# peach-xiao/EMRT

Measured on AMD Instinct MI355X. Metric: training tiles/sec at 256x256, higher is better.
Workload: dtype bf16; 1 GPU; EMRT ResNet50, Potsdam 256x256, 6 classes, batch 8 per GPU, fwd+bwd+SGD step (BASELINE configs[1]), bf16; global_batch=8, parallelism=dp1, hipgraph=True

## Files before the change

__graft_entry__.py:

```python
import os
import sys

ROOT = os.path.dirname(os.path.abspath(__file__))
if ROOT not in sys.path:
    sys.path.insert(0, ROOT)


def build():
    from emrt_amd import build_ext
    lib = build_ext.build()
    import emrt_amd
    from emrt_amd import _lib
    L = _lib.lib()
    assert L.query("emrt_abi_version") == 9
    A = _lib.augment_lib()
    assert A.query("emrt_aug_version") == 1
    S = _lib.sampler_lib()
    assert S.query("emrt_smp_version") == 1
    X = _lib.loss_lib()
    assert X.query("emrt_lx_version") == 1
    print("[build] %s: %d entry points" % (os.path.relpath(build_ext.AUG_LIB, ROOT), len(A.protos)))
    print("[build] %s: %d entry points" % (os.path.relpath(build_ext.SMP_LIB, ROOT), len(S.protos)))
    print("[build] %s: %d entry points" % (os.path.relpath(build_ext.LOSS_LIB, ROOT), len(X.protos)))
    print("[build] %s: %d entry points; build mode: %s (%s); inputs sha256 %s" % (
        os.path.relpath(lib, ROOT), len(L.protos), build_ext.LAST_BUILD["mode"],
        ", ".join(build_ext.LAST_BUILD["compiled"]) or "no source changed since the objects were built", build_ext.LAST_BUILD["digest"][:16]))


def smoke():
    import torch
    from emrt_amd.runtime import F32
    from emrt_amd.src.models.emrt import EMRT
    from emrt_amd.src.models.losses import MixSoftmaxCrossEntropyLoss
    from emrt_amd.src.models.solver import Momentum, PolynomialDecay
    from oracle.emrt_torch import EMRT as OracleEMRT

    torch.manual_seed(0)
    ref = OracleEMRT(6, "resnet18").eval()
    model = EMRT(num_classes=6, backbone="resnet18")
    model.load_state_dict(ref.state_dict())
    model.to_hip("cuda:0", F32)
    x = torch.randn(2, 3, 64, 64)
    labels = torch.randint(0, 6, (2, 64, 64))
    model.eval()
    got = model(x.cuda())[0].cpu()
    with torch.no_grad():
        want = ref(x)[0]
    err = (got - want).abs().max().item()
    assert err < 1e-3, "HIP forward differs from the oracle: max |diff| = %g" % err
    assert torch.equal(got.argmax(1), want.argmax(1)), "argmax masks differ from the oracle"
    model.train()
    opt = Momentum(model, PolynomialDecay(0.01, 1000), 0.9, 1e-4, 1.0)
    loss_fn = MixSoftmaxCrossEntropyLoss(ignore_index=255, aux=True, aux_weight=0.4)
    model.clear_gradients()
    loss = loss_fn(model(x.cuda()), labels.cuda())
    loss.backward()
    opt.step()
    torch.cuda.synchronize()
    val = loss.item()
    assert val == val and val > 0, "bad loss %r" % val
    print("[smoke] ok: forward max|diff| vs oracle %.3g, train-step loss %.4f, grad norm %.4f" % (err, val, opt.grad_norm()))


if __name__ == "__main__":
    build()
    if "--smoke" in sys.argv:
        smoke()
```

emrt_amd/_lib.py:

```python
import ctypes
import keyword
import os
import re

_HERE = os.path.dirname(os.path.abspath(__file__))
HEADER = os.path.join(os.path.dirname(_HERE), "include", "emrt_hip.h")
LIB_PATH = os.environ.get("EMRT_HIP_LIB") or os.path.join(_HERE, "csrc", "libemrt_hip.so")

AUG_HEADER = os.path.join(os.path.dirname(_HERE), "include", "emrt_hip_augment.h")
AUG_LIB_PATH = os.environ.get("EMRT_HIP_AUGMENT_LIB") or os.path.join(_HERE, "csrc", "libemrt_hip_augment.so")

SMP_HEADER = os.path.join(os.path.dirname(_HERE), "include", "emrt_hip_sampler.h")
SMP_LIB_PATH = os.environ.get("EMRT_HIP_SAMPLER_LIB") or os.path.join(_HERE, "csrc", "libemrt_hip_sampler.so")

LOSS_HEADER = os.path.join(os.path.dirname(_HERE), "include", "emrt_hip_loss.h")
LOSS_LIB_PATH = os.environ.get("EMRT_HIP_LOSS_LIB") or os.path.join(_HERE, "csrc", "libemrt_hip_loss.so")

_TRACE = bool(int(os.environ.get("EMRT_TRACE", "0")))

_CTYPES = {
    "int": ctypes.c_int, "unsigned": ctypes.c_uint, "float": ctypes.c_float, "double": ctypes.c_double,
    "long long": ctypes.c_longlong, "size_t": ctypes.c_size_t,
}

# ... 248 lines not shown
            setattr(self, "_raw_" + name, fn)
        self._last_error = getattr(self, "_raw_%s_last_error" % prefix)
        version = getattr(self, "_raw_%s_version" % prefix)()
        if version != 1:
            raise EmrtHipError("%s has version %d, this binding expects 1" % (so, version))

    def last_error(self):
        return self._last_error().decode("utf-8", "replace")

    def call(self, name, *args):
        if _TRACE:
            print("[emrt] %s%r" % (name, tuple(a.value if hasattr(a, "value") else a for a in args)), flush=True)
        rc = getattr(self, "_raw_" + name)(*args)
        if rc != 0:
            raise EmrtHipError("%s failed (%d): %s" % (name, rc, self.last_error()))
        if _TRACE:
            import torch
            torch.cuda.synchronize()

    def query(self, name, *args):
        return getattr(self, "_raw_" + name)(*args)


_AUG_LIB = None


def augment_lib():
    global _AUG_LIB
    if _AUG_LIB is None:
        _AUG_LIB = _ExtLib(AUG_LIB_PATH, AUG_HEADER, "emrt_aug", "the device augmentation")
    return _AUG_LIB



_SMP_LIB = None


def sampler_lib():
    global _SMP_LIB
    if _SMP_LIB is None:
        _SMP_LIB = _ExtLib(SMP_LIB_PATH, SMP_HEADER, "emrt_smp", "the class-aware scene sampler")
    return _SMP_LIB



_LOSS_LIB = None


def loss_lib():
    global _LOSS_LIB
    if _LOSS_LIB is None:
        _LOSS_LIB = _ExtLib(LOSS_LIB_PATH, LOSS_HEADER, "emrt_lx", "the Dice + cross-entropy loss")
    return _LOSS_LIB
```

emrt_amd/build_ext.py:

```python
import os
import subprocess
import sys
from concurrent.futures import ThreadPoolExecutor

HERE = os.path.dirname(os.path.abspath(__file__))
CSRC = os.path.join(HERE, "csrc")
LIB = os.path.join(CSRC, "libemrt_hip.so")
SOURCES = ["conv.hip", "norm.hip", "msda.hip", "attn.hip", "spatial.hip", "loss.hip", "optim.hip", "elementwise.hip", "gconv.hip", "augment.hip", "scene.hip"]
HEADER = os.path.join(os.path.dirname(HERE), "include", "emrt_hip.h")
AUG_DIR = os.path.join(CSRC, "augment_ext")
AUG_LIB = os.path.join(CSRC, "libemrt_hip_augment.so")
AUG_SOURCES = ["augment_ext.hip"]
AUG_HEADER = os.path.join(os.path.dirname(HERE), "include", "emrt_hip_augment.h")
SMP_DIR = os.path.join(CSRC, "sampler_ext")
SMP_LIB = os.path.join(CSRC, "libemrt_hip_sampler.so")
SMP_SOURCES = ["sampler_ext.hip"]
SMP_HEADER = os.path.join(os.path.dirname(HERE), "include", "emrt_hip_sampler.h")
GROUPS = [(LIB, CSRC, SOURCES, HEADER), (AUG_LIB, AUG_DIR, AUG_SOURCES, AUG_HEADER), (SMP_LIB, SMP_DIR, SMP_SOURCES, SMP_HEADER)]
LOSS_DIR = os.path.join(CSRC, "loss_ext")
LOSS_LIB = os.path.join(CSRC, "libemrt_hip_loss.so")
LOSS_SOURCES = ["loss_ext.hip"]
LOSS_HEADER = os.path.join(os.path.dirname(HERE), "include", "emrt_hip_loss.h")
EXTRA_GROUPS = [(LOSS_LIB, LOSS_DIR, LOSS_SOURCES, LOSS_HEADER)]
FLAGS = ["--offload-arch=gfx950", "-O3", "-std=c++17", "-fPIC", "-munsafe-fp-atomics", "-Wno-unused-result", "-I../../include"]


def _hipcc():
    for cand in (os.environ.get("HIPCC"), "/opt/rocm/bin/hipcc", "hipcc"):
        if cand and (os.path.isabs(cand) and os.path.exists(cand) or not os.path.isabs(cand)):
            return cand
    return "hipcc"


def _digest(paths, extra=()):
    import hashlib
    h = hashlib.sha256()
    for e in extra:
        h.update(str(e).encode() + b"\0")
    for p in paths:
        h.update(os.path.basename(p).encode() + b"\0")
        with open(p, "rb") as f:
            h.update(f.read())
        h.update(b"\0")
    return h.hexdigest()


def _stamp(target):
    return target + ".inputs"


def _fresh(target, digest):
    try:
        with open(_stamp(target)) as f:
            return os.path.exists(target) and f.read().strip() == digest
    except OSError:
        return False


def all_groups():
    return GROUPS + EXTRA_GROUPS


def _headers():
    return [os.path.join(CSRC, h) for h in sorted(os.listdir(CSRC)) if h.endswith(".hpp")] + [g[3] for g in all_groups()]


def source_digest():
    return _digest([os.path.join(d, s) for _, d, sources, _ in all_groups() for s in sources] + _headers(), [_hipcc()] + FLAGS)


LAST_BUILD = {"mode": None, "digest": None, "compiled": [], "linked": []}


def build(force=False, verbose=True):
    hipcc = _hipcc()
    hdrs = _headers()
    objs, jobs = {g[0]: [] for g in all_groups()}, []
    for lib, d, sources, _ in all_groups():
        for src in sources:
            s = os.path.join(d, src)
            o = os.path.join(d, src.replace(".hip", ".o"))
            objs[lib].append(o)
            dg = _digest([s] + hdrs, [hipcc] + FLAGS)
            if force or not _fresh(o, dg):
                jobs.append(([hipcc] + FLAGS + ["-c", s, "-o", o], o, dg, lib))

    def run(cmd):
        r = subprocess.run(cmd, capture_output=True, text=True, cwd=CSRC)
        if r.returncode != 0:
            raise RuntimeError("hipcc failed: %s\n%s" % (" ".join(cmd), r.stderr[-4000:]))

    def compile_one(job):
        cmd, o, d, _ = job
        if os.path.exists(_stamp(o)):
            os.remove(_stamp(o))
        run(cmd)
        with open(_stamp(o), "w") as f:
            f.write(d + "\n")
        return cmd[-3]

    LAST_BUILD["compiled"] = []
    for lib in {j[3] for j in jobs}:
        if os.path.exists(_stamp(lib)):
            os.remove(_stamp(lib))
    if jobs:
        with ThreadPoolExecutor(max_workers=min(4, len(jobs))) as ex:
            for done in ex.map(compile_one, jobs):
                LAST_BUILD["compiled"].append(os.path.basename(done))
                if verbose:
                    print("[emrt_amd.build] compiled", os.path.basename(done), flush=True)
    total = source_digest()
    linked = LAST_BUILD["linked"] = []
    for lib, _, _, _ in all_groups():
# ... 20 lines not shown
```

emrt_amd/functional.py:

```python
import ctypes
import math

import torch

from . import _lib
from .runtime import ctx, dtype_of, F32


def _L():
    return _lib.lib()


def P(t):
    return None if t is None else ctypes.c_void_p(t.data_ptr())


def _check_map(t):
    assert t.stride(-1) == 1, "inner stride must be 1: %s %s" % (tuple(t.shape), t.stride())
    if t.dim() == 4:
        N, H, W, C = t.shape
        ld = t.stride(2) if W > 1 else (t.stride(1) if H > 1 else (t.stride(0) if N > 1 else C))
        assert H == 1 or W == 1 or t.stride(1) == W * t.stride(2), \
            "expected an NHWC view with dense rows, got shape %s strides %s" % (tuple(t.shape), t.stride())
        return N, H, W, C, ld, (t.stride(0) if N > 1 else H * W * ld)
# ... 6 lines not shown
def _like_shape(t, C):
    return tuple(t.shape[:-1]) + (C,)


def _rows(t):
    C = t.shape[-1]
    assert t.stride(-1) == 1
    ld = t.stride(-2) if t.dim() >= 2 else C
    rows = t.numel() // C
    for d in range(t.dim() - 2):
        assert t.stride(d) == t.stride(d + 1) * t.shape[d + 1], "rows are not uniformly strided: %s %s" % (tuple(t.shape), t.stride())
    return rows, C, ld


def tokens_as_map(t, h, w):
    B, n, C = t.shape
    assert n == h * w
    v = t.as_strided((B, h, w, C), (t.stride(0), w * t.stride(1), t.stride(1), 1), t.storage_offset())
    tape = ctx().tape
    if tape is not None:
        tape.register_alias(v, t, lambda g: g.as_strided((B, h, w, C), (g.stride(0), w * g.stride(1), g.stride(1), 1), g.storage_offset()))
    return v


def map_as_tokens(t):
    B, h, w, C = t.shape
    assert t.stride(1) == w * t.stride(2)
    v = t.as_strided((B, h * w, C), (t.stride(0), t.stride(2), 1), t.storage_offset())
    tape = ctx().tape
    if tape is not None:
        tape.register_alias(v, t, lambda g: g.as_strided((B, h * w, C), (g.stride(0), g.stride(2), 1), g.storage_offset()))
    return v


def view_as(t, shape):
    v = t.view(shape)
    tape = ctx().tape
    if tape is not None:
        tape.register_alias(v, t, lambda g: g.view(shape))
    return v


def param_input(p_data, p_grad):
    c = ctx()
    t = cast_from_f32(p_data)
    tape = c.tape
    if tape is not None:
        def bwd():
            g = tape.pop_grad(t)
            if g is not None:
                add_into(p_grad, cast_to_f32(g))
        tape.record(bwd)
    return t


def narrow(t, dim, start, length):
    v = t.narrow(dim, start, length)
    tape = ctx().tape
    if tape is not None:
        tape.register_alias(v, t, lambda g: g.narrow(dim, start, length))
    return v


def _geom3(*tensors):
    n = tensors[0].numel()
    split = None
    for t in tensors:
        assert t.numel() == n
        if t.dim() >= 2 and not t.is_contiguous():
            N, H, W, C, ld, bs = _check_map(t)
            cur = (N, H * W, C)
            assert split is None or split == cur, "incompatible views %s vs %s" % (split, cur)
            split = cur
    if split is None:
        split = (1, 1, n)
    B, R, Cc = split
    strides = []
    for t in tensors:
        if t.dim() >= 2 and not t.is_contiguous():
            _, _, _, _, ld, bs = _check_map(t)
            strides.append((bs, ld))
        else:
            strides.append((R * Cc, Cc))
    return B, R, Cc, strides


def add_into(dst, src):
    c = ctx()
    assert dst.dtype == src.dtype, (dst.dtype, src.dtype)
    dt = dtype_of(dst)
    B, R, Cc, (sd, ss) = _geom3(dst, src)
    _L().call("emrt_acc3d", P(dst), sd[0], sd[1], P(src), ss[0], ss[1], B, R, Cc, dt, c.stream)


def add(a, b, period=None, bgrad=None):
    c = ctx()
    assert a.is_contiguous() and b.is_contiguous()
    out = c.empty(tuple(a.shape), a.dtype)
    n = a.numel()
    per = n if period is None else period
    dt = dtype_of(a)
    _L().call("emrt_add", P(a), P(b), P(out), n, per, dt, c.stream)
    tape = c.tape
    if tape is not None:
        def bwd():
            g = tape.pop_grad(out)
# ... 1138 lines not shown
    rows = a.numel() // C
    out = c.empty(tuple(a.shape))
    q = None
    if q_pos is not None:
        assert q_pos.is_contiguous() and q_pos.dtype == a.dtype and q_pos.shape[-1] == C and rows % (q_pos.numel() // C) == 0
        q = c.empty(tuple(a.shape))
    keep = c.tape is not None
    p = float(drop_p) if (c.training and b is not None) else 0.0
    z = c.empty(tuple(a.shape)) if (keep and b is not None) else None
    mean = c.empty((rows,), torch.float32) if keep else None
    rstd = c.empty((rows,), torch.float32) if keep else None
    _L().call("emrt_layernorm_fwd", P(a), P(b), P(post), P(z), P(out), P(gamma), P(beta), P(mean), P(rstd), rows, C, eps, p,
              c.seed_ptr if p > 0 else None, drop_salt, P(q_pos) if q is not None else None, (q_pos.numel() // C) if q is not None else 0, P(q),
              c.dtype, c.stream)
    tape = c.tape
    if tape is not None:
        zz = z if z is not None else a

        def bwd():
            dy = tape.pop_grad(out)
            dq = tape.pop_grad(q) if q is not None else None
            if dq is not None:
                assert dq.is_contiguous() and dq.dtype == out.dtype
                if q_bgrad is not None:
                    q_bgrad(dq)
                if dy is None:
                    dy, dq = dq, None
            if dy is None:
                return
            assert dy.is_contiguous()
            dz = c.empty(tuple(a.shape))
            dzb = c.empty(tuple(a.shape)) if (b is not None and p > 0) else None
            ws = c.workspace(_L().query("emrt_layernorm_bwd_workspace_bytes", rows, C))
            dysum = c.empty(tuple(a.shape)) if (dq is not None and post is not None) else None
            extra = tape.peek_grad(identity_from) if identity_from is not None else None
            if extra is not None and (not extra.is_contiguous() or tuple(extra.shape) != tuple(a.shape) or extra.dtype != dz.dtype or (b is not None and dzb is None)):
                extra = None
            _L().call("emrt_layernorm_bwd", P(zz), P(dy), P(dz), P(gamma), P(mean), P(rstd), P(dgamma), P(dbeta), rows, C, P(ws), P(dzb), p,
                      c.seed_ptr if p > 0 else None, drop_salt, P(extra), P(dq), P(dysum), c.dtype, c.stream)
            if extra is not None:
                tape.identity_done[id(identity_from)] = (extra, tape.grad_count(identity_from))
            tape.add_grad(a, dz, owned=(b is None or dzb is not None))
            if b is not None:
                if dzb is not None:
                    tape.add_grad(b, dzb, owned=True)
                else:
                    tape.add_grad(b, dz)
            if post is not None:
                tape.add_grad(post, dy if dysum is None else dysum, owned=dysum is not None)
        tape.record(bwd)
    return out if q is None else (out, q)


def msda(value, offw, ref, shapes, n_heads, n_points, need_dref=False):
    c = ctx()
    B, Lv, CC = value.shape
    M, L, Pn = n_heads, len(shapes), n_points
    assert CC == M * 32 and value.stride(2) == 1
    Lq, ldo = offw.shape[1], offw.shape[2]
    assert offw.is_contiguous() and offw.dtype == torch.float32 and ref.dtype == torch.float32 and ref.is_contiguous()
    ref_L = ref.shape[2]
    assert ref.shape[1] == Lq and ref_L in (1, L) and ref.shape[3] == 2
    ref_bs = 0 if ref.shape[0] == 1 else Lq * ref_L * 2
    arr = (ctypes.c_int * (2 * L))(*[int(v) for hw in shapes for v in hw])
    out = c.empty((B, Lq, CC))
    _L().call("emrt_msda_fwd", P(value), value.stride(1), value.stride(0), P(offw), ldo, P(ref), ref_bs, ref_L, P(out), B, Lq, Lv, M, 32, L, Pn,
              ctypes.cast(arr, ctypes.c_void_p), c.dtype, c.stream)
    tape = c.tape
    if tape is not None:
        def bwd():
            dy = tape.pop_grad(out)
            if dy is None:
                return
            assert dy.is_contiguous()
            odt = None if c.dtype != F32 else torch.float32
            doffw = c.zeros((B, Lq, ldo), odt) if ldo != M * L * Pn * 3 else c.empty((B, Lq, ldo), odt)
            dref = c.zeros((B, Lq, ref_L, 2), torch.float32) if need_dref else None
            dvalue = c.empty((B, Lv, CC))
            ws = c.empty((_L().query("emrt_msda_bwd_workspace_bytes", B, Lq, M, L, Pn, ctypes.cast(arr, ctypes.c_void_p), c.dtype) // 4,), torch.float32)
            _L().call("emrt_msda_bwd", P(value), value.stride(1), value.stride(0), P(offw), ldo, P(ref), ref_bs, ref_L, P(dy), P(dvalue), P(doffw),
                      int(c.dtype != F32), P(dref), B, Lq, Lv, M, 32, L, Pn, ctypes.cast(arr, ctypes.c_void_p), P(ws), ws.numel() * 4, c.dtype, c.stream)
            tape.add_grad(value, dvalue, owned=True)
            tape.add_grad(offw, doffw, owned=True)
            if need_dref:
                if ref.shape[0] == 1 and B > 1:
                    red = c.zeros((1, Lq, ref_L, 2), torch.float32)
                    colsum_acc(dref.view(B, Lq * ref_L * 2), red.view(-1))
                    dref = red
                tape.add_grad(ref, dref)
        tape.record(bwd)
    return out


def mha(qk, v, n_heads, pdrop, salt):
    c = ctx()
    B, L, E2 = qk.shape
    E = E2 // 2
    assert qk.is_contiguous() and v.is_contiguous() and E == n_heads * 32
    out = c.empty((B, L, E))
    probs = c.empty((B, n_heads, L, L), torch.float32)
    p = float(pdrop) if c.training else 0.0
    scale = 1.0 / math.sqrt(32.0)
    q_ptr = qk.data_ptr()
    k_ptr = qk.data_ptr() + E * qk.element_size()
    path = ctypes.c_int(-1)
    _L().call("emrt_mha_fwd", ctypes.c_void_p(q_ptr), E2, ctypes.c_void_p(k_ptr), E2, P(v), E, P(out), E, P(probs), B, n_heads, L, 32, scale, p,
              c.seed_ptr, salt, ctypes.pointer(path), c.dtype, c.stream)
    tape = c.tape
    if tape is not None:
        def bwd():
            dy = tape.pop_grad(out)
            if dy is None:
                return
            assert dy.is_contiguous()
            dqk = c.empty((B, L, E2))
            dv = c.empty((B, L, E))
            _L().call("emrt_mha_bwd", ctypes.c_void_p(q_ptr), E2, ctypes.c_void_p(k_ptr), E2, P(v), E, P(probs), P(dy), E,
                      ctypes.c_void_p(dqk.data_ptr()), E2, ctypes.c_void_p(dqk.data_ptr() + E * dqk.element_size()), E2, P(dv), E,
                      B, n_heads, L, 32, scale, p, c.seed_ptr, salt, path.value, c.dtype, c.stream)
            tape.add_grad(qk, dqk, owned=True)
            tape.add_grad(v, dv, owned=True)
        tape.record(bwd)
    return out


def nchw_to_nhwc(img, c_out=None):
    c = ctx()
    N, C, H, W = img.shape
    assert img.dtype == torch.float32 and img.is_contiguous()
    co = C if c_out is None else int(c_out)
    out = c.empty((N, H, W, co))
    _L().call("emrt_nchw_to_nhwc", P(img), P(out), N, C, H, W, co, c.dtype, c.stream)
    return out


def resize_bilinear(x, OH, OW, align_corners, add_t=None, out=None, out_nchw_f32=False):
    c = ctx()
# ... 372 lines not shown
```

emrt_amd/runtime.py:

```python
import ctypes

import torch

from . import _lib

F32, BF16, F16 = 0, 1, 2
_TORCH_DTYPE = {F32: torch.float32, BF16: torch.bfloat16, F16: torch.float16}
_DTYPE_OF_TORCH = {v: k for k, v in _TORCH_DTYPE.items()}


def dtype_of(t):
    return _DTYPE_OF_TORCH[t.dtype]


class Tape:
    def __init__(self):
        self.ops = []
        self.stash = None
        self.grads = {}
        self.keep = []
        self.alias = {}
        self.watched = {}
        self.results = {}
        self.splits = []
# ... 142 lines not shown
            _CTX.wgrad_join()
        finally:
            _CTX._in_backward = False
        if stop_at > 0:
            return
        self.results = {k: self.grad(t) for k, t in self.watched.items()}
        self.ops = []
        self.grads = {}
        self.keep = []
        self.alias = {}
        self.identity_done = {}


class Context:
    def __init__(self):
        self.dtype = F32
        self.tape = None
        self.training = False
        self.device = None
        self._ws = None
        self._seed = None
        self.step_counter = None
        self.world_size = 1
        self.sync_bn = True
        self.salt_counter = 0
        self.keepalive = None
        self._arena = None
        self._arena_off = 0
        self._arena_live = False
        self.overlap = False
        self._side = None
        self._in_backward = False
        self._main = None
        self.fold_eval_bn = True
        self.fold_live = False
        self.capture = None
        self.sync_always = False
        import os
        self.wgrad_batch = int(os.environ.get("EMRT_WGRAD_BATCH", "24"))
        self.bn_defer = bool(int(os.environ.get("EMRT_BN_DEFER", "1")))
        self.bn_conv = bool(int(os.environ.get("EMRT_BN_CONV", "1")))
        self.bn_small_group = bool(int(os.environ.get("EMRT_BN_SMALL_GROUP", "1")))
        self.conv_pair = bool(int(os.environ.get("EMRT_CONV_PAIR", "1")))
        self.side_branch = bool(int(os.environ.get("EMRT_SIDE_BRANCH", "1")))
        self.side = None
        self.dgrad_pair = bool(int(os.environ.get("EMRT_DGRAD_PAIR", "1")))
        self.side_host_tiles = int(os.environ.get("EMRT_SIDE_HOST_TILES", "128"))
        self.segment_order = False
        self.head_pair = bool(int(os.environ.get("EMRT_HEAD_PAIR", "1")))
        self.enc_front = bool(int(os.environ.get("EMRT_ENC_FRONT", "1")))
        self.group_attn_proj = bool(int(os.environ.get("EMRT_GROUP_ATTN_PROJ", "1")))
        self.fuse_ffn_dropout = bool(int(os.environ.get("EMRT_FFN_DROPOUT_FUSED", "1")))
        self.ln_query = bool(int(os.environ.get("EMRT_LN_QUERY", "1")))
        self.pyramid_group = bool(int(os.environ.get("EMRT_PYRAMID_GROUP", "1")))
        self.wgrad_side = bool(int(os.environ.get("EMRT_WGRAD_SIDE", "0")))
        self._wside = None
        self._wside_keep = []
        self.prologue_side = bool(int(os.environ.get("EMRT_PROLOGUE_SIDE", "0")))
        self._pside = None
        self._prologue_pending = False
        self.pack_bwd_done = False

    def collective(self, fn):
        self.prologue_join()
        if self.capture is not None:
            self.capture.interlude(fn)
        else:
            fn()

    def prologue_stream(self):
        if self._pside is None:
            self._pside = torch.cuda.Stream(device=self.device)
        self._pside.wait_stream(torch.cuda.current_stream())
        self._prologue_pending = True
        return self._pside

    def prologue_join(self):
        if self._prologue_pending:
            torch.cuda.current_stream().wait_stream(self._pside)
            self._prologue_pending = False

    def fork(self, *keep):
        if not self.overlap:
            return None
        if self._side is None:
            self._side = torch.cuda.Stream(device=self.device)
            self._side_keep = []
        self._side.wait_stream(torch.cuda.current_stream())
        if self.overlap == "deferred":
            self._side_keep.extend(keep)
        return ctypes.c_void_p(self._side.cuda_stream)

    def join(self):
        if self.overlap == "pair":
            torch.cuda.current_stream().wait_stream(self._side)

    def join_all(self):
        if self._side is not None:
            torch.cuda.current_stream().wait_stream(self._side)
            self._side_keep = []
        self.wgrad_join()

    def wgrad_fork(self, keep):
        if self._wside is None:
            self._wside = torch.cuda.Stream(device=self.device)
        self._wside.wait_stream(torch.cuda.current_stream())
# ... 133 lines not shown
```

emrt_amd/src/models/emrt.py:

```python
import ctypes
import math

import torch
import torch.nn as tnn

from ... import functional as Fn
from ... import nn as hnn
from ...runtime import ctx, Tape, F32

NOGRAD_PARAMS = ("backbone.fc.weight", "backbone.fc.bias", "model.tgt_embed.weight", "backbone.out.weight", "backbone.out.bias")
IMAGE_CHANNELS = 8

LATE_GRAD_PREFIXES = ("backbone.conv1.", "backbone.bn1.", "backbone.layer1.", "backbone.layer2.", "backbone.layer3.")
GRAD_SEGMENT_PREFIXES = (("backbone.layer3.",), ("backbone.conv1.", "backbone.bn1.", "backbone.layer1.", "backbone.layer2."))


def _salt():
    return ctx().next_salt()


class BasicBlock(hnn.HipLayer):
    expansion = 1

    def __init__(self, inplanes, planes, stride=1, downsample=None):
# ... 220 lines not shown
    def __init__(self, in_channels, channels, num_classes, dropout_ratio=0.1, up_ratio=16):
        super().__init__()
        self.up_ratio, self.p = up_ratio, dropout_ratio
        self.convs = hnn.Sequential(hnn.Sequential(hnn.Conv2D(in_channels, channels, 3, 1, 1, bias=False),
                                                   hnn.BatchNorm2D(channels, sync=True), None))
        self.conv_seg = hnn.Conv2D(channels, num_classes, 1)
        self.salt = _salt()

    def forward(self, x, features=None):
        N, H, W, _ = x.shape
        o = features if features is not None else Fn.conv_bn(self.convs[0][0], self.convs[0][1], x, relu=True)
        o = Fn.dropout(o, self.p, self.salt, mode=1, hw=H * W, sole_consumer_is_linear=True)
        o = self.conv_seg(o)
        return Fn.resize_bilinear(o, H * self.up_ratio, W * self.up_ratio, False, out_nchw_f32=True)


class MSDeformableAttention(hnn.HipLayer):
    def __init__(self, embed_dim=256, num_heads=8, num_levels=3, num_points=6):
        super().__init__()
        self.embed_dim, self.num_heads, self.num_levels, self.num_points = embed_dim, num_heads, num_levels, num_points
        tp = num_heads * num_levels * num_points
        self.total_points = tp
        self.sampling_offsets = hnn.Linear(embed_dim, tp * 2)
        self.attention_weights = hnn.Linear(embed_dim, tp)
        self.value_proj = hnn.Linear(embed_dim, embed_dim)
        self.output_proj = hnn.Linear(embed_dim, embed_dim)
        self.sampling_offsets.standalone = False
        self.attention_weights.standalone = False
        self.offw_gemm = None
        self._reset_parameters()

    @torch.no_grad()
    def _reset_parameters(self):
        tnn.init.zeros_(self.sampling_offsets.weight)
        thetas = torch.arange(self.num_heads, dtype=torch.float32) * (2.0 * math.pi / self.num_heads)
        grid = torch.stack([thetas.cos(), thetas.sin()], -1)
        grid = grid / grid.abs().max(-1, keepdim=True)[0]
        grid = grid.reshape(self.num_heads, 1, 1, 2).repeat(1, self.num_levels, self.num_points, 1)
        grid = grid * torch.arange(1, self.num_points + 1, dtype=torch.float32).reshape(1, 1, -1, 1)
        self.sampling_offsets.bias.copy_(grid.flatten())
        tnn.init.zeros_(self.attention_weights.weight)
        tnn.init.zeros_(self.attention_weights.bias)
        tnn.init.xavier_uniform_(self.value_proj.weight)
        tnn.init.zeros_(self.value_proj.bias)
        tnn.init.xavier_uniform_(self.output_proj.weight)
        tnn.init.zeros_(self.output_proj.bias)

    def bind(self, store, prefix):
        ow, ob = store.offsets[prefix + "sampling_offsets.weight"], store.offsets[prefix + "sampling_offsets.bias"]
        assert store.offsets[prefix + "attention_weights.weight"] == ow + self.total_points * 2 * self.embed_dim
        assert store.offsets[prefix + "attention_weights.bias"] == ob + self.total_points * 2
        self.offw_gemm = store.make_gemm(ow, self.total_points * 3, self.embed_dim, 1, 1, ob)

    def forward(self, query, reference_points, value, spatial_shapes, need_dref=False, projected=None):
        c = ctx()
        if projected is not None:
            value, offw = projected
        elif c.group_attn_proj and value.dim() == 3 and query.dim() == 3 and value.is_contiguous() and query.is_contiguous() and value is not query:
            value, offw = Fn.linear_group([(value, self.value_proj.gw, False), (query, self.offw_gemm, True)])
        else:
            value = self.value_proj(value)
            offw = Fn.linear(query, self.offw_gemm, out_f32=True)
        out = Fn.msda(value, offw, reference_points, spatial_shapes, self.num_heads, self.num_points, need_dref=need_dref)
        return self.output_proj(out)


class MultiHeadAttention(hnn.HipLayer):
    def __init__(self, embed_dim, num_heads, dropout=0.0):
        super().__init__()
        self.embed_dim, self.num_heads, self.dropout = embed_dim, num_heads, dropout
        self.in_proj_weight = tnn.Parameter(torch.empty(3 * embed_dim, embed_dim))
        self.in_proj_bias = tnn.Parameter(torch.zeros(3 * embed_dim))
        self.out_proj = hnn.Linear(embed_dim, embed_dim)
        self.salt = _salt()
        with torch.no_grad():
            bound = math.sqrt(6.0 / (embed_dim + 3 * embed_dim))
            self.in_proj_weight.uniform_(-bound, bound)
            tnn.init.xavier_uniform_(self.out_proj.weight)
            tnn.init.zeros_(self.out_proj.bias)

    def bind(self, store, prefix):
        E = self.embed_dim
        w, b = store.offsets[prefix + "in_proj_weight"], store.offsets[prefix + "in_proj_bias"]
        self.qk_gemm = store.make_gemm(w, 2 * E, E, 1, 1, b)
        self.v_gemm = store.make_gemm(w + 2 * E * E, E, E, 1, 1, b + 2 * E)

    def forward(self, qk_in, v_in):
        if ctx().group_attn_proj and qk_in.is_contiguous() and v_in.is_contiguous() and qk_in.dim() == 3:
            qk, v = Fn.linear_group([(qk_in, self.qk_gemm, False), (v_in, self.v_gemm, False)])
        else:
            qk = Fn.linear(qk_in, self.qk_gemm)
            v = Fn.linear(v_in, self.v_gemm)
        out = Fn.mha(qk, v, self.num_heads, self.dropout, self.salt)
        return self.out_proj(out)


def _linear_init_(m):
    bound = 1 / math.sqrt(m.weight.shape[1])
    tnn.init.uniform_(m.weight, -bound, bound)
    tnn.init.uniform_(m.bias, -bound, bound)


@torch.no_grad()
def _paddle_conv_default_(conv):
    fan = conv.weight.shape[1] * conv.weight.shape[2] * conv.weight.shape[3]
    conv.weight.normal_(0.0, math.sqrt(2.0 / fan))
    if conv.bias is not None:
        conv.bias.zero_()


class TransformerEncoderLayer(hnn.HipLayer):
    def __init__(self, d_model=256, n_head=8, dim_feedforward=1024, dropout=0.1, n_levels=3, n_points=6):
        super().__init__()
        self.p = dropout
        self.self_attn = MSDeformableAttention(d_model, n_head, n_levels, n_points)
        self.norm1 = hnn.LayerNorm(d_model)
# ... 24 lines not shown
                q = Fn.add(src, pos, period=Lv * C, bgrad=pos_bgrad)
            lin = [(src, self.self_attn.value_proj.gw, False), (q, self.self_attn.offw_gemm, True)]
            if c.enc_front and c.group_attn_proj and q.is_contiguous() and q is not src and Fn.level_conv_gn_takes_linears(src, gws, lin):
                src_flatten, projected = Fn.level_conv_gn(src, gws, gns, spatial_shapes, level_spans, linears=lin)
            else:
                src_flatten = Fn.level_conv_gn(src, gws, gns, spatial_shapes, level_spans)
            identity = src_flatten
        else:
            identity = None
            src_flatten = ctx().empty((B, Lv, C))
            for (h, w), (s0, n), seq in zip(spatial_shapes, level_spans, seqs):
                x_l = Fn.tokens_as_map(Fn.narrow(src, 1, s0, n), h, w)
                y = seq[0](x_l)
                seq[1](y, gelu=True, residual=x_l, out=Fn.tokens_as_map(Fn.narrow(src_flatten, 1, s0, n), h, w))
        if q is None:
            q = Fn.add(src, pos, period=Lv * C, bgrad=pos_bgrad)
        src2 = self.self_attn(q, reference_points, src, spatial_shapes, projected=projected)
        src = self.norm1(src, src2, drop_p=self.p, drop_salt=self.salts[0], identity_from=identity)
        h1 = self.linear1(src, relu=True, drop=(self.p, self.salts[1]))
        ff = self.linear2(h1)
        return self.norm2(src, ff, post=src_flatten, drop_p=self.p, drop_salt=self.salts[2], q_pos=pos if next_q else None, q_bgrad=pos_bgrad)


class TransformerEncoder(hnn.HipLayer):
    def __init__(self, make_layer, num_layers):
        super().__init__()
        first = make_layer()
        layers = [first]
        for _ in range(1, num_layers):
            lyr = make_layer()
            lyr.load_state_dict(first.state_dict())
            layers.append(lyr)
        self.layers = tnn.ModuleList(layers)


class TransformerDecoderLayer(hnn.HipLayer):
    def __init__(self, d_model=256, n_head=8, dim_feedforward=1024, dropout=0.1, n_levels=3, n_points=6):
        super().__init__()
        self.p = dropout
        self.self_attn = MultiHeadAttention(d_model, n_head, dropout=dropout)
        self.norm1 = hnn.LayerNorm(d_model)
        self.cross_attn = MSDeformableAttention(d_model, n_head, n_levels, n_points)
        self.norm2 = hnn.LayerNorm(d_model)
        self.linear1 = hnn.Linear(d_model, dim_feedforward)
        self.linear2 = hnn.Linear(dim_feedforward, d_model)
        self.norm3 = hnn.LayerNorm(d_model)
        self.salts = [_salt(), _salt(), _salt(), _salt()]
        with torch.no_grad():
            _linear_init_(self.linear1)
            _linear_init_(self.linear2)
            tnn.init.xavier_uniform_(self.linear1.weight)
            tnn.init.xavier_uniform_(self.linear2.weight)

    def forward(self, tgt, reference_points, memory, spatial_shapes, query_pos, qpos_bgrad, q=None, next_q=False):
        Lq, C = tgt.shape[1], tgt.shape[2]
        fuse = ctx().ln_query
        if q is None:
            q = Fn.add(tgt, query_pos, period=Lq * C, bgrad=qpos_bgrad)
        if fuse:
            tgt, q2 = self.norm1(tgt, self.self_attn(q, tgt), drop_p=self.p, drop_salt=self.salts[0], q_pos=query_pos, q_bgrad=qpos_bgrad)
        else:
            tgt = self.norm1(tgt, self.self_attn(q, tgt), drop_p=self.p, drop_salt=self.salts[0])
            q2 = Fn.add(tgt, query_pos, period=Lq * C, bgrad=qpos_bgrad)
        tgt2 = self.cross_attn(q2, reference_points, memory, spatial_shapes, need_dref=True)
        tgt = self.norm2(tgt, tgt2, drop_p=self.p, drop_salt=self.salts[1])
        h1 = self.linear1(tgt, relu=True, drop=(self.p, self.salts[2]))
        return self.norm3(tgt, self.linear2(h1), drop_p=self.p, drop_salt=self.salts[3], q_pos=query_pos if next_q else None, q_bgrad=qpos_bgrad)


class TransformerDecoder(hnn.HipLayer):
    def __init__(self, make_layer, num_layers):
        super().__init__()
        first = make_layer()
        layers = [first]
        for _ in range(1, num_layers):
            lyr = make_layer()
            lyr.load_state_dict(first.state_dict())
            layers.append(lyr)
        self.layers = tnn.ModuleList(layers)


def sine_position_embedding(h, w, num_pos_feats=128, temperature=10000, offset=-0.5, eps=1e-6, scale=2 * math.pi):
    y_embed = torch.arange(1, h + 1, dtype=torch.float32).reshape(h, 1).expand(h, w)
    x_embed = torch.arange(1, w + 1, dtype=torch.float32).reshape(1, w).expand(h, w)
    y_embed = (y_embed + offset) / (y_embed[-1:, :] + eps) * scale
    x_embed = (x_embed + offset) / (x_embed[:, -1:] + eps) * scale
    dim_t = 2 * (torch.arange(num_pos_feats) // 2).to(torch.float32)
    dim_t = temperature ** (dim_t / num_pos_feats)
    pos_x = x_embed.unsqueeze(-1) / dim_t
    pos_y = y_embed.unsqueeze(-1) / dim_t
    pos_x = torch.stack((pos_x[:, :, 0::2].sin(), pos_x[:, :, 1::2].cos()), dim=3).flatten(2)
    pos_y = torch.stack((pos_y[:, :, 0::2].sin(), pos_y[:, :, 1::2].cos()), dim=3).flatten(2)
    return torch.cat((pos_y, pos_x), dim=2).reshape(h * w, 2 * num_pos_feats)


def encoder_reference_points(spatial_shapes):
    pts = []
    for (H, W) in spatial_shapes:
        ref_y, ref_x = torch.meshgrid(torch.linspace(0.5, H - 0.5, H), torch.linspace(0.5, W - 0.5, W), indexing="ij")
        pts.append(torch.stack((ref_x.flatten() / W, ref_y.flatten() / H), dim=-1))
    return torch.cat(pts, 0).reshape(1, -1, 1, 2).contiguous()


class EncoderDecoder(hnn.HipLayer):
    def __init__(self, num_queries=110, backbone_num_channels=(512, 1024, 2048), num_feature_levels=3,
                 num_encoder_points=6, num_decoder_points=6, hidden_dim=256, nhead=8, num_encoder_layers=4,
                 num_decoder_layers=2, dim_feedforward=1024, dropout=0.1):
        super().__init__()
        self.hidden_dim, self.nhead, self.num_queries = hidden_dim, nhead, num_queries
        self.encoder = TransformerEncoder(lambda: TransformerEncoderLayer(hidden_dim, nhead, dim_feedforward, dropout,
                                                                          num_feature_levels, num_encoder_points), num_encoder_layers)
        self.decoder = TransformerDecoder(lambda: TransformerDecoderLayer(hidden_dim, nhead, dim_feedforward, dropout,
                                                                          num_feature_levels, num_decoder_points), num_decoder_layers)
        self.level_embed = hnn.Embedding(num_feature_levels, hidden_dim)
        self.tgt_embed = hnn.Embedding(num_queries, hidden_dim)
        self.query_pos_embed = hnn.Embedding(num_queries, hidden_dim)
        self.reference_points = hnn.Linear(hidden_dim, 2)
# ... 27 lines not shown
        spans, s0 = [], 0
        for h, w in spatial_shapes:
            spans.append((s0, h * w))
            s0 += h * w
        Lv = s0
        if all(f.is_contiguous() and n <= 4096 for f, (_, n) in zip(src_feats, spans)) and len(src_feats) <= 4:
            src, _ = Fn.level_proj_gn(list(src_feats), [p_[0].gw for p_ in self.input_proj],
                                      [(p_[1].weight.data, p_[1].bias.data, p_[1].weight.grad, p_[1].bias.grad) for p_ in self.input_proj])
        else:
            src = c.empty((B, Lv, C))
            for f, (h, w), (a, n), proj in zip(src_feats, spatial_shapes, spans, self.input_proj):
                y = proj[0](f)
                proj[1](y, out=Fn.tokens_as_map(Fn.narrow(src, 1, a, n), h, w))
        sine, ref_enc = self._constants(spatial_shapes)
        pos = c.empty((Lv, C))
        lvl = self.level_embed.weight
        if len(spans) <= 4 and lvl.data.is_contiguous():
            starts = (ctypes.c_int * len(spans))(*[a for a, _ in spans])
            Fn._L().call("emrt_add_f32row_levels", Fn.P(sine), Fn.P(lvl.data), Fn.P(pos), starts, len(spans), Lv, C, c.dtype, c.stream)
        else:
            for l, (a, n) in enumerate(spans):
                Fn._L().call("emrt_add_f32row", Fn.P(sine[a:a + n]), Fn.P(lvl.data[l]), Fn.P(pos[a:a + n]), n * C, C, c.dtype, c.stream)

        pos_acc = []

        def pos_bgrad(g):
            pos_acc.append(g)

        if c.tape is not None:
            def pos_reduce():
                if not pos_acc:
                    return
                if (len(pos_acc) <= 8 and len(spans) <= 4 and all(g.is_contiguous() and tuple(g.shape) == (B, Lv, C) and g.dtype == pos_acc[0].dtype for g in pos_acc)
                        and lvl.grad.is_contiguous() and C % 4 == 0 and 256 % (C // 4) == 0):
                    ptrs = (ctypes.c_void_p * len(pos_acc))(*[g.data_ptr() for g in pos_acc])
                    st_ = (ctypes.c_int * len(spans))(*[a for a, _ in spans])
                    cn_ = (ctypes.c_int * len(spans))(*[n for _, n in spans])
                    Fn._L().call("emrt_colsum_levels_multi", ptrs, len(pos_acc), st_, cn_, len(spans), B, Lv, C, Fn.P(lvl.grad), Fn.dtype_of(pos_acc[0]), c.stream)
                else:
                    for g in pos_acc:
                        for l, (a, n) in enumerate(spans):
                            Fn.colsum_acc(g.narrow(1, a, n), lvl.grad[l])
                pos_acc.clear()
            c.tape.record(pos_reduce)

        memory, q = src, None
        n_enc = len(self.encoder.layers)
        for i, layer in enumerate(self.encoder.layers):
            nq = c.ln_query and i + 1 < n_enc
            res = layer(memory, ref_enc, spatial_shapes, spans, pos, pos_bgrad, q=q, next_q=nq)
            memory, q = res if nq else (res, None)

        qpe = self.query_pos_embed.weight
        query_pos = Fn.param_input(qpe.data, qpe.grad)

        def qpos_bgrad(g):
            Fn.colsum_acc(g.reshape(g.shape[0], -1), qpe.grad.view(-1))

        ref_logit = self.reference_points(query_pos, out_f32=True)
        ref_dec = Fn.view_as(Fn.sigmoid_f32(ref_logit), (1, self.num_queries, 1, 2))
        tgt, q = src_psp, None
        n_dec = len(self.decoder.layers)
        for i, layer in enumerate(self.decoder.layers):
            nq = c.ln_query and i + 1 < n_dec
            res = layer(tgt, ref_dec, memory, spatial_shapes, query_pos, qpos_bgrad, q=q, next_q=nq)
            tgt, q = res if nq else (res, None)
        return tgt, memory, spatial_shapes, spans


class Conv2dBlock(hnn.HipLayer):
    def __init__(self, cin, cout):
        super().__init__()
        self.conv1 = hnn.Sequential(hnn.Conv2D(cin, cout, 3, 1, 1, bias=False), hnn.BatchNorm2D(cout), None)
        self.conv2 = hnn.Sequential(hnn.Conv2D(cout, cout, 3, 1, 1, bias=False), hnn.BatchNorm2D(cout), None)

    def forward(self, x):
        o = Fn.conv_bn(self.conv1[0], self.conv1[1], x, relu=True, defer="conv")
        o = Fn.conv_bn(self.conv2[0], self.conv2[1], o, relu=True)
        return Fn.add_maps(o, x)


class EFP(hnn.HipLayer):
    def __init__(self, cin=256, cout=256):
        super().__init__()
        self.conv0, self.conv1, self.conv2 = Conv2dBlock(cin, cout), Conv2dBlock(cin, cout), Conv2dBlock(cin, cout)

    def forward(self, x0, x1, x2, out):
        blocks, xs = (self.conv0, self.conv1, self.conv2), (x0, x1, x2)
        c1, b1 = [b.conv1[0] for b in blocks], [b.conv1[1] for b in blocks]
        c2, b2 = [b.conv2[0] for b in blocks], [b.conv2[1] for b in blocks]
        if Fn._small_group_ok(c1, b1, xs):
            mid = Fn.conv_bn_small_group(c1, b1, xs, relu=True)
            if Fn._small_group_ok(c2, b2, mid, post_adds=xs):
                o0, o1, o2 = Fn.conv_bn_small_group(c2, b2, mid, relu=True, post_adds=xs)
            else:
                o0, o1, o2 = [Fn.add_maps(Fn.conv_bn(cv, b, m_, relu=True), x) for cv, b, m_, x in zip(c2, b2, mid, xs)]
            x21 = Fn.resize_bilinear(o2, x1.shape[1], x1.shape[2], True, add_t=o1)
            return Fn.resize_bilinear(x21, x0.shape[1], x0.shape[2], True, add_t=o0, out=out)
        o2 = self.conv2(x2)
        o1 = self.conv1(x1)
        x21 = Fn.resize_bilinear(o2, x1.shape[1], x1.shape[2], True, add_t=o1)
        o0 = self.conv0(x0)
        return Fn.resize_bilinear(x21, x0.shape[1], x0.shape[2], True, add_t=o0, out=out)


class PyramidPoolingModule(hnn.HipLayer):
    def __init__(self, pool_scales, in_channels, channels):
        super().__init__()
        self.pool_scales = list(pool_scales)
        self.pool_branches = tnn.ModuleList([
            hnn.Sequential(None, hnn.Conv2D(in_channels, channels, 1, bias=False), hnn.BatchNorm2D(channels, sync=True), None)
            for _ in pool_scales])

    def forward(self, x, extra=None):
        tokens = Fn.adaptive_avgpool_tokens(x, self.pool_scales)
        slices, s0 = [], 0
        for k in self.pool_scales:
            slices.append(Fn.narrow(tokens, 1, s0, k * k))
# ... 249 lines not shown
```

Baseline: 1011 tiles/s.

## Fuse decoder query-pos cast, reference-point linear and sigmoid into one kernel

Adds a new HIP extension that, in one forward kernel, casts the query-position embedding, computes the 2-wide reference-point projection and applies the sigmoid. The backward pass collects the query-pos gradient slabs and MSDA reference-point gradients from all decoder layers and reduces them in one kernel, instead of a colsum per layer plus separate linear and sigmoid backward passes. It is meant to remove several small launches and the per-layer dref reductions. The cost is more code, buffered gradient lists that flush when full, and a fallback path for unsupported shapes.

Result: no change. 1018 tiles/s (median of 6 runs) (+0.7%).

```diff
diff --git a/__graft_entry__.py b/__graft_entry__.py
--- a/__graft_entry__.py
+++ b/__graft_entry__.py
@@ -19,9 +19,12 @@
     assert S.query("emrt_smp_version") == 1
     X = _lib.loss_lib()
     assert X.query("emrt_lx_version") == 1
+    Y = _lib.query_lib()
+    assert Y.query("emrt_qp_version") == 1
     print("[build] %s: %d entry points" % (os.path.relpath(build_ext.AUG_LIB, ROOT), len(A.protos)))
     print("[build] %s: %d entry points" % (os.path.relpath(build_ext.SMP_LIB, ROOT), len(S.protos)))
     print("[build] %s: %d entry points" % (os.path.relpath(build_ext.LOSS_LIB, ROOT), len(X.protos)))
+    print("[build] %s: %d entry points" % (os.path.relpath(build_ext.QUERY_LIB, ROOT), len(Y.protos)))
     print("[build] %s: %d entry points; build mode: %s (%s); inputs sha256 %s" % (
         os.path.relpath(lib, ROOT), len(L.protos), build_ext.LAST_BUILD["mode"],
         ", ".join(build_ext.LAST_BUILD["compiled"]) or "no source changed since the objects were built", build_ext.LAST_BUILD["digest"][:16]))
diff --git a/emrt_amd/_lib.py b/emrt_amd/_lib.py
--- a/emrt_amd/_lib.py
+++ b/emrt_amd/_lib.py
@@ -324,3 +324,17 @@
     if _LOSS_LIB is None:
         _LOSS_LIB = _ExtLib(LOSS_LIB_PATH, LOSS_HEADER, "emrt_lx", "the Dice + cross-entropy loss")
     return _LOSS_LIB
+
+
+
+QUERY_HEADER = os.path.join(os.path.dirname(_HERE), "include", "emrt_hip_query.h")
+QUERY_LIB_PATH = os.environ.get("EMRT_HIP_QUERY_LIB") or os.path.join(_HERE, "csrc", "libemrt_hip_query.so")
+
+_QUERY_LIB = None
+
+
+def query_lib():
+    global _QUERY_LIB
+    if _QUERY_LIB is None:
+        _QUERY_LIB = _ExtLib(QUERY_LIB_PATH, QUERY_HEADER, "emrt_qp", "the decoder's query parameters")
+    return _QUERY_LIB
diff --git a/emrt_amd/build_ext.py b/emrt_amd/build_ext.py
--- a/emrt_amd/build_ext.py
+++ b/emrt_amd/build_ext.py
@@ -22,6 +22,11 @@
 LOSS_SOURCES = ["loss_ext.hip"]
 LOSS_HEADER = os.path.join(os.path.dirname(HERE), "include", "emrt_hip_loss.h")
 EXTRA_GROUPS = [(LOSS_LIB, LOSS_DIR, LOSS_SOURCES, LOSS_HEADER)]
+QUERY_DIR = os.path.join(CSRC, "query_ext")
+QUERY_LIB = os.path.join(CSRC, "libemrt_hip_query.so")
+QUERY_SOURCES = ["query_ext.hip"]
+QUERY_HEADER = os.path.join(os.path.dirname(HERE), "include", "emrt_hip_query.h")
+MORE_GROUPS = [(QUERY_LIB, QUERY_DIR, QUERY_SOURCES, QUERY_HEADER)]
 FLAGS = ["--offload-arch=gfx950", "-O3", "-std=c++17", "-fPIC", "-munsafe-fp-atomics", "-Wno-unused-result", "-I../../include"]
 
 
@@ -58,7 +63,7 @@
 
 
 def all_groups():
-    return GROUPS + EXTRA_GROUPS
+    return GROUPS + EXTRA_GROUPS + MORE_GROUPS
 
 
 def _headers():
diff --git a/emrt_amd/csrc/query_ext/query_ext.hip b/emrt_amd/csrc/query_ext/query_ext.hip
--- /dev/null
+++ b/emrt_amd/csrc/query_ext/query_ext.hip
@@ -0,0 +1,173 @@
+#include "../common.hpp"
+#include "../../../include/emrt_hip_query.h"
+
+namespace emrt {
+namespace {
+
+thread_local char g_qp_err[512] = "";
+
+int qp_fail(const char* fn, const char* msg) {
+  snprintf(g_qp_err, sizeof(g_qp_err), "%s: %s", fn, msg);
+  return -1;
+}
+int qp_check_launch(const char* fn) {
+  hipError_t e = hipGetLastError();
+  if (e != hipSuccess) {
+    snprintf(g_qp_err, sizeof(g_qp_err), "%s: launch failed: %s", fn, hipGetErrorString(e));
+    return -2;
+  }
+  return 0;
+}
+#define QP_REQUIRE(cond, msg)                     \
+  do {                                            \
+    if (!(cond)) return qp_fail(__func__, msg);   \
+  } while (0)
+
+}
+
+template <class T>
+__device__ __forceinline__ float rounded(float x) { return to_f32(from_f32<T>(x)); }
+
+template <class T>
+__global__ __launch_bounds__(256) void qp_prep_fwd_kernel(const float* __restrict__ embed, const float* __restrict__ weight, const float* __restrict__ bias,
+                                                          T* __restrict__ query_pos, float* __restrict__ ref, int Q, int C) {
+  const int lane = threadIdx.x & 63, q = blockIdx.x * 4 + (threadIdx.x >> 6);
+  if (q >= Q) return;
+  float a0 = 0.f, a1 = 0.f;
+  for (int c = lane; c < C; c += 64) {
+    const T xt = from_f32<T>(embed[(size_t)q * C + c]);
+    query_pos[(size_t)q * C + c] = xt;
+    const float x = to_f32(xt);
+    a0 = fmaf(x, rounded<T>(weight[c]), a0);
+    a1 = fmaf(x, rounded<T>(weight[C + c]), a1);
+  }
+  a0 = wave_sum(a0);
+  a1 = wave_sum(a1);
+  if (lane < 2) {
+    const float z = (lane ? a1 : a0) + (bias ? bias[lane] : 0.f);
+    ref[q * 2 + lane] = 1.f / (1.f + expf(-z));
+  }
+}
+
+template <class T>
+struct QpBwd {
+  const T* slab[EMRT_QP_MAX_SLABS];
+  const float* dref[EMRT_QP_MAX_DREF];
+  int nslabs, ndref;
+  const float* ref;
+  const T* query_pos;
+  const float* weight;
+  float *d_embed, *d_weight, *d_bias;
+  int B, Q, C, row_blocks;
+};
+
+template <class T>
+__device__ __forceinline__ float qp_dlogit(const QpBwd<T>& a, int q, int j) {
+  float s = 0.f;
+  for (int k = 0; k < a.ndref; ++k)
+    for (int b = 0; b < a.B; ++b) s += a.dref[k][((size_t)b * a.Q + q) * 2 + j];
+  const float r = a.ref[q * 2 + j];
+  return s * r * (1.f - r);
+}
+
+template <class T>
+__global__ __launch_bounds__(256) void qp_prep_bwd_kernel(QpBwd<T> a) {
+  __shared__ float dl[EMRT_QP_MAX_QUERIES * 2];
+  __shared__ float part[4][2][64];
+  const int lane = threadIdx.x & 63, wv = threadIdx.x >> 6;
+  const int Q = a.Q, C = a.C;
+  if ((int)blockIdx.x < a.row_blocks) {
+    const int q = blockIdx.x * 4 + wv;
+    if (q >= Q) return;
+    const float d0 = qp_dlogit(a, q, 0), d1 = qp_dlogit(a, q, 1);
+    for (int c = lane * 4; c < C; c += 256) {
+      float acc[4] = {0.f, 0.f, 0.f, 0.f};
+      for (int s = 0; s < a.nslabs; ++s) {
+        const T* g = a.slab[s] + (size_t)q * C + c;
+#pragma unroll 4
+        for (int b = 0; b < a.B; ++b) {
+          float v[4];
+          Vec4<T>::load(g + (size_t)b * Q * C, v);
+#pragma unroll
+          for (int e = 0; e < 4; ++e) acc[e] += v[e];
+        }
+      }
+#pragma unroll
+      for (int e = 0; e < 4; ++e) {
+        float t = fmaf(d0, rounded<T>(a.weight[c + e]), acc[e]);
+        t = fmaf(d1, rounded<T>(a.weight[C + c + e]), t);
+        a.d_embed[(size_t)q * C + c + e] += t;
+      }
+    }
+    return;
+  }
+  for (int i = threadIdx.x; i < 2 * Q; i += 256) dl[i] = qp_dlogit(a, i >> 1, i & 1);
+  __syncthreads();
+  const int c = ((int)blockIdx.x - a.row_blocks) * 64 + lane;
+  float w0 = 0.f, w1 = 0.f;
+  if (c < C) {
+    for (int q = wv; q < Q; q += 4) {
+      const float x = to_f32(a.query_pos[(size_t)q * C + c]);
+      w0 = fmaf(dl[q * 2], x, w0);
+      w1 = fmaf(dl[q * 2 + 1], x, w1);
+    }
+  }
+  part[wv][0][lane] = w0;
+  part[wv][1][lane] = w1;
+  __syncthreads();
+  if (wv < 2 && c < C)
+    a.d_weight[(size_t)wv * C + c] += ((part[0][wv][lane] + part[1][wv][lane]) + part[2][wv][lane]) + part[3][wv][lane];
+  if ((int)blockIdx.x == a.row_blocks && wv == 2 && a.d_bias) {
+    float b0 = 0.f, b1 = 0.f;
+    for (int q = lane; q < Q; q += 64) { b0 += dl[q * 2]; b1 += dl[q * 2 + 1]; }
+    b0 = wave_sum(b0);
+    b1 = wave_sum(b1);
+    if (lane < 2) a.d_bias[lane] += lane ? b1 : b0;
+  }
+}
+
+}
+
+using namespace emrt;
+
+extern "C" const char* emrt_qp_last_error(void) { return g_qp_err; }
+extern "C" int emrt_qp_version(void) { return 1; }
+
+extern "C" int emrt_qp_prep_fwd(const float* embed, const float* weight, const float* bias, void* query_pos, float* ref, int Q, int C, int dtype, void* stream) {
+  QP_REQUIRE(dtype == EMRT_F32 || dtype == EMRT_BF16 || dtype == EMRT_F16, "dtype must be 0 (float32), 1 (bfloat16) or 2 (float16)");
+  QP_REQUIRE(embed && weight && query_pos && ref, "null pointer");
+  QP_REQUIRE(Q >= 1 && Q <= EMRT_QP_MAX_QUERIES && C >= 1 && C <= 65536, "1 <= Q <= 2048 and 1 <= C <= 65536");
+  const dim3 grid((unsigned)((Q + 3) / 4));
+  hipStream_t st = (hipStream_t)stream;
+  if (dtype == EMRT_F32) hipLaunchKernelGGL(qp_prep_fwd_kernel<float>, grid, dim3(256), 0, st, embed, weight, bias, (float*)query_pos, ref, Q, C);
+  else if (dtype == EMRT_BF16) hipLaunchKernelGGL(qp_prep_fwd_kernel<bf16_t>, grid, dim3(256), 0, st, embed, weight, bias, (bf16_t*)query_pos, ref, Q, C);
+  else hipLaunchKernelGGL(qp_prep_fwd_kernel<f16_t>, grid, dim3(256), 0, st, embed, weight, bias, (f16_t*)query_pos, ref, Q, C);
+  return qp_check_launch("emrt_qp_prep_fwd");
+}
+
+template <class T>
+static int qp_backward(const void* const* slabs, int nslabs, const float* const* drefs, int ndref, const float* ref, const void* query_pos, const float* weight,
+                       float* d_embed, float* d_weight, float* d_bias, int B, int Q, int C, void* stream) {
+  QpBwd<T> a;
+  for (int s = 0; s < EMRT_QP_MAX_SLABS; ++s) a.slab[s] = s < nslabs ? (const T*)slabs[s] : nullptr;
+  for (int s = 0; s < EMRT_QP_MAX_DREF; ++s) a.dref[s] = s < ndref ? drefs[s] : nullptr;
+  a.nslabs = nslabs; a.ndref = ndref; a.ref = ref; a.query_pos = (const T*)query_pos; a.weight = weight;
+  a.d_embed = d_embed; a.d_weight = d_weight; a.d_bias = d_bias;
+  a.B = B; a.Q = Q; a.C = C; a.row_blocks = (Q + 3) / 4;
+  hipLaunchKernelGGL(qp_prep_bwd_kernel<T>, dim3((unsigned)(a.row_blocks + (C + 63) / 64)), dim3(256), 0, (hipStream_t)stream, a);
+  return qp_check_launch("emrt_qp_prep_bwd");
+}
+
+extern "C" int emrt_qp_prep_bwd(const void* slabs, int nslabs, const void* drefs, int ndref, const float* ref, const void* query_pos, const float* weight,
+                                float* d_embed, float* d_weight, float* d_bias, int B, int Q, int C, int dtype, void* stream) {
+  QP_REQUIRE(dtype == EMRT_F32 || dtype == EMRT_BF16, "dtype must be 0 (float32) or 1 (bfloat16): float16 is inference-only");
+  QP_REQUIRE(nslabs >= 0 && nslabs <= EMRT_QP_MAX_SLABS && ndref >= 0 && ndref <= EMRT_QP_MAX_DREF, "0..8 gradient slabs and 0..4 reference-point gradients");
+  QP_REQUIRE((slabs || nslabs == 0) && (drefs || ndref == 0) && ref && query_pos && weight && d_embed && d_weight, "null pointer");
+  QP_REQUIRE(B >= 1 && Q >= 1 && Q <= EMRT_QP_MAX_QUERIES && C >= 4 && C <= 65536 && C % 4 == 0, "B >= 1, 1 <= Q <= 2048, 4 <= C <= 65536 and C % 4 == 0");
+  const void* const* sl = (const void* const*)slabs;
+  const float* const* dr = (const float* const*)drefs;
+  for (int s = 0; s < nslabs; ++s) QP_REQUIRE(sl[s] && ((uintptr_t)sl[s]) % 16 == 0, "every gradient slab must be a 16-byte aligned device pointer");
+  for (int s = 0; s < ndref; ++s) QP_REQUIRE(dr[s], "null reference-point gradient");
+  if (dtype == EMRT_F32) return qp_backward<float>(sl, nslabs, dr, ndref, ref, query_pos, weight, d_embed, d_weight, d_bias, B, Q, C, stream);
+  return qp_backward<bf16_t>(sl, nslabs, dr, ndref, ref, query_pos, weight, d_embed, d_weight, d_bias, B, Q, C, stream);
+}
diff --git a/emrt_amd/functional.py b/emrt_amd/functional.py
--- a/emrt_amd/functional.py
+++ b/emrt_amd/functional.py
@@ -82,6 +82,43 @@
                 add_into(p_grad, cast_to_f32(g))
         tape.record(bwd)
     return t
+
+
+def query_prep(embed, weight, bias):
+    c = ctx()
+    Q, C = embed.data.shape
+    assert tuple(weight.data.shape) == (2, C) and embed.data.is_contiguous() and weight.data.is_contiguous()
+    X = _lib.query_lib()
+    query_pos = c.empty((Q, C))
+    ref = c.empty((Q, 2), torch.float32)
+    X.call("emrt_qp_prep_fwd", P(embed.data), P(weight.data), P(bias.data if bias is not None else None), P(query_pos), P(ref), Q, C, c.dtype, c.stream)
+    slabs, drefs = [], []
+    tape = c.tape
+    if tape is not None:
+        def flush():
+            B = (slabs[0] if slabs else drefs[0]).shape[0]
+            assert all(g.is_contiguous() and tuple(g.shape) == (B, Q, C) and g.dtype == query_pos.dtype for g in slabs)
+            assert all(d.is_contiguous() and tuple(d.shape) == (B, Q, 1, 2) and d.dtype == torch.float32 for d in drefs)
+            sp = (ctypes.c_void_p * max(len(slabs), 1))(*[g.data_ptr() for g in slabs])
+            dp = (ctypes.c_void_p * max(len(drefs), 1))(*[d.data_ptr() for d in drefs])
+            X.call("emrt_qp_prep_bwd", sp, len(slabs), dp, len(drefs), P(ref), P(query_pos), P(weight.data), P(embed.grad), P(weight.grad),
+                   P(bias.grad if bias is not None else None), B, Q, C, c.dtype, c.stream)
+            slabs.clear()
+            drefs.clear()
+
+        def add(lst, cap):
+            def sink(g):
+                if len(lst) == cap:
+                    flush()
+                lst.append(g)
+            return sink
+
+        def bwd():
+            if slabs or drefs:
+                flush()
+        tape.record(bwd)
+        return query_pos, ref, add(slabs, 8), add(drefs, 4)
+    return query_pos, ref, None, None
 
 
 def narrow(t, dim, start, length):
@@ -1326,7 +1363,7 @@
     return out if q is None else (out, q)
 
 
-def msda(value, offw, ref, shapes, n_heads, n_points, need_dref=False):
+def msda(value, offw, ref, shapes, n_heads, n_points, need_dref=False, dref_sink=None):
     c = ctx()
     B, Lv, CC = value.shape
     M, L, Pn = n_heads, len(shapes), n_points
@@ -1356,7 +1393,9 @@
                       int(c.dtype != F32), P(dref), B, Lq, Lv, M, 32, L, Pn, ctypes.cast(arr, ctypes.c_void_p), P(ws), ws.numel() * 4, c.dtype, c.stream)
             tape.add_grad(value, dvalue, owned=True)
             tape.add_grad(offw, doffw, owned=True)
-            if need_dref:
+            if need_dref and dref_sink is not None:
+                dref_sink(dref)
+            elif need_dref:
                 if ref.shape[0] == 1 and B > 1:
                     red = c.zeros((1, Lq, ref_L, 2), torch.float32)
                     colsum_acc(dref.view(B, Lq * ref_L * 2), red.view(-1))
diff --git a/emrt_amd/runtime.py b/emrt_amd/runtime.py
--- a/emrt_amd/runtime.py
+++ b/emrt_amd/runtime.py
@@ -218,6 +218,7 @@
         self.group_attn_proj = bool(int(os.environ.get("EMRT_GROUP_ATTN_PROJ", "1")))
         self.fuse_ffn_dropout = bool(int(os.environ.get("EMRT_FFN_DROPOUT_FUSED", "1")))
         self.ln_query = bool(int(os.environ.get("EMRT_LN_QUERY", "1")))
+        self.query_prep = bool(int(os.environ.get("EMRT_QUERY_PREP", "1")))
         self.pyramid_group = bool(int(os.environ.get("EMRT_PYRAMID_GROUP", "1")))
         self.wgrad_side = bool(int(os.environ.get("EMRT_WGRAD_SIDE", "0")))
         self._wside = None
diff --git a/emrt_amd/src/models/emrt.py b/emrt_amd/src/models/emrt.py
--- a/emrt_amd/src/models/emrt.py
+++ b/emrt_amd/src/models/emrt.py
@@ -296,7 +296,7 @@
         assert store.offsets[prefix + "attention_weights.bias"] == ob + self.total_points * 2
         self.offw_gemm = store.make_gemm(ow, self.total_points * 3, self.embed_dim, 1, 1, ob)
 
-    def forward(self, query, reference_points, value, spatial_shapes, need_dref=False, projected=None):
+    def forward(self, query, reference_points, value, spatial_shapes, need_dref=False, projected=None, dref_sink=None):
         c = ctx()
         if projected is not None:
             value, offw = projected
@@ -305,7 +305,7 @@
         else:
             value = self.value_proj(value)
             offw = Fn.linear(query, self.offw_gemm, out_f32=True)
-        out = Fn.msda(value, offw, reference_points, spatial_shapes, self.num_heads, self.num_points, need_dref=need_dref)
+        out = Fn.msda(value, offw, reference_points, spatial_shapes, self.num_heads, self.num_points, need_dref=need_dref, dref_sink=dref_sink)
         return self.output_proj(out)
 
 
@@ -436,7 +436,7 @@
             tnn.init.xavier_uniform_(self.linear1.weight)
             tnn.init.xavier_uniform_(self.linear2.weight)
 
-    def forward(self, tgt, reference_points, memory, spatial_shapes, query_pos, qpos_bgrad, q=None, next_q=False):
+    def forward(self, tgt, reference_points, memory, spatial_shapes, query_pos, qpos_bgrad, q=None, next_q=False, dref_sink=None):
         Lq, C = tgt.shape[1], tgt.shape[2]
         fuse = ctx().ln_query
         if q is None:
@@ -446,7 +446,7 @@
         else:
             tgt = self.norm1(tgt, self.self_attn(q, tgt), drop_p=self.p, drop_salt=self.salts[0])
             q2 = Fn.add(tgt, query_pos, period=Lq * C, bgrad=qpos_bgrad)
-        tgt2 = self.cross_attn(q2, reference_points, memory, spatial_shapes, need_dref=True)
+        tgt2 = self.cross_attn(q2, reference_points, memory, spatial_shapes, need_dref=True, dref_sink=dref_sink)
         tgt = self.norm2(tgt, tgt2, drop_p=self.p, drop_salt=self.salts[1])
         h1 = self.linear1(tgt, relu=True, drop=(self.p, self.salts[2]))
         return self.norm3(tgt, self.linear2(h1), drop_p=self.p, drop_salt=self.salts[3], q_pos=query_pos if next_q else None, q_bgrad=qpos_bgrad)
@@ -580,18 +580,25 @@
             memory, q = res if nq else (res, None)
 
         qpe = self.query_pos_embed.weight
-        query_pos = Fn.param_input(qpe.data, qpe.grad)
-
-        def qpos_bgrad(g):
-            Fn.colsum_acc(g.reshape(g.shape[0], -1), qpe.grad.view(-1))
-
-        ref_logit = self.reference_points(query_pos, out_f32=True)
-        ref_dec = Fn.view_as(Fn.sigmoid_f32(ref_logit), (1, self.num_queries, 1, 2))
+        rp = self.reference_points
+        dref_sink = None
+        if (c.query_prep and C % 4 == 0 and self.num_queries <= 2048 and qpe.data.is_cuda and qpe.data.is_contiguous() and rp.weight.data.is_contiguous()
+                and rp.bias is not None):
+            query_pos, ref, qpos_bgrad, dref_sink = Fn.query_prep(qpe, rp.weight, rp.bias)
+            ref_dec = ref.view(1, self.num_queries, 1, 2)
+        else:
+            query_pos = Fn.param_input(qpe.data, qpe.grad)
+
+            def qpos_bgrad(g):
+                Fn.colsum_acc(g.reshape(g.shape[0], -1), qpe.grad.view(-1))
+
+            ref_logit = rp(query_pos, out_f32=True)
+            ref_dec = Fn.view_as(Fn.sigmoid_f32(ref_logit), (1, self.num_queries, 1, 2))
         tgt, q = src_psp, None
         n_dec = len(self.decoder.layers)
         for i, layer in enumerate(self.decoder.layers):
             nq = c.ln_query and i + 1 < n_dec
-            res = layer(tgt, ref_dec, memory, spatial_shapes, query_pos, qpos_bgrad, q=q, next_q=nq)
+            res = layer(tgt, ref_dec, memory, spatial_shapes, query_pos, qpos_bgrad, q=q, next_q=nq, dref_sink=dref_sink)
             tgt, q = res if nq else (res, None)
         return tgt, memory, spatial_shapes, spans
 
diff --git a/include/emrt_hip_query.h b/include/emrt_hip_query.h
--- /dev/null
+++ b/include/emrt_hip_query.h
@@ -0,0 +1,23 @@
+#ifndef EMRT_HIP_QUERY_H
+#define EMRT_HIP_QUERY_H
+#include <stddef.h>
+
+#ifdef __cplusplus
+extern "C" {
+#endif
+
+#define EMRT_QP_MAX_SLABS 8
+#define EMRT_QP_MAX_DREF 4
+#define EMRT_QP_MAX_QUERIES 2048
+
+const char* emrt_qp_last_error(void);
+int emrt_qp_version(void);
+
+int emrt_qp_prep_fwd(const float* embed, const float* weight, const float* bias, void* query_pos, float* ref, int Q, int C, int dtype, void* stream);
+
+int emrt_qp_prep_bwd(const void* slabs, int nslabs, const void* drefs, int ndref, const float* ref, const void* query_pos, const float* weight, float* d_embed, float* d_weight, float* d_bias, int B, int Q, int C, int dtype, void* stream);
+
+#ifdef __cplusplus
+}
+#endif
+#endif
```
